# lmb-freiburg/flownet2

Hardware: AMD Instinct MI355X
Metric: image-pairs/sec FlowNetC forward at 448x320 (higher is better)
Workload: dtype f32

## Files before the change

flownet2_amd/csrc/conv_mfma.hip:

```cpp
#include "mfma_tile.hpp"

namespace fn2 {
namespace cv {

using namespace mfma;

struct Args {
  const float* in; const float* wp; const float* bias; float* out;
  int N, Cin, Hin, Win, in_ctot, in_c0;
  int Cout, Hout, Wout, out_ctot, out_c0;
  int pad;
  int nchunks;
  int ksteps;
  int tx, ty;
  int ng;
  unsigned total;
  unsigned nbig;
  float slope; int relu;
};

template <int KS_, int S_, int MW_, int NP_, int WM_, int WNX_, int WNY_, int CQ_, int P16_ = 0, int PIN_ = 0>
struct Cfg : Window<((P16_ ? 1 : 4) * WNY_ - 1) * S_ + KS_,
                    ((P16_ ? 16 : 4) * NP_ * WNX_ - 1) * S_ + KS_ + 4,
                    CQ_, WM_ * WNX_ * WNY_> {
  static constexpr int KS = KS_, S = S_, MW = MW_, NP = NP_, WM = WM_, WNX = WNX_, WNY = WNY_, CQ = CQ_, P16 = P16_;
  static constexpr int PIN = PIN_;
  static constexpr int NW = WM * WNX * WNY, THREADS = 64 * NW;
  static constexpr int PADL = 4;
  static constexpr int TW = (P16 ? 16 : 4) * NP * WNX, TH = (P16 ? 1 : 4) * WNY;
  static_assert(!P16 || (KS == 1 && S == 1), "row tiles are for 1x1 kernels");
  static_assert(Cfg::WR == (TH - 1) * S + KS && Cfg::WC == (TW - 1) * S + KS + PADL, "window of the tile");
  static constexpr int KSC = CQ * KS * KS;
  static constexpr int NBUFA = ring_depth(KSC);
  static_assert(KSC % NBUFA == 0, "ring phase must repeat per chunk");
  static_assert(2 * Cfg::BUF * 4 <= 160 * 1024, "LDS");
};

template <class K>
__device__ __forceinline__ void conv_body(const Args& a, int g, int bx, int by, int n) {
  static_assert(K::THREADS == 256, "launch bounds");
  extern __shared__ __attribute__((aligned(16))) float smem[];
  constexpr int KS = K::KS, S = K::S, MW = K::MW, NP = K::NP;
  const int tid = threadIdx.x, lane = tid & 63;
  const int wave = __builtin_amdgcn_readfirstlane(tid >> 6);
  const int wm = wave % K::WM, wnx = (wave / K::WM) % K::WNX, wny = wave / (K::WM * K::WNX);
  const int x0 = bx * K::TW, y0 = by * K::TH;

  const size_t plane = (size_t)a.Hin * a.Win;
  const __amdgpu_buffer_rsrc_t rs = nchw_rsrc(a.in, n, a.in_ctot, a.in_c0, a.Cin, plane);
  unsigned voff[K::RPW];
  window_plan<K>(voff, wave, lane, S * y0 - a.pad, S * x0 - K::PADL, a.Hin, a.Win, plane);
  const unsigned lds_base = (unsigned)(uintptr_t)(lds_ptr_t)smem;
  const unsigned chunk_bytes = 4u * 4u * K::CQ * (unsigned)plane;
  auto stage = [&](int chunk, int buf) { stage_chunk<K>(rs, voff, lds_base + 4u * (unsigned)(buf * K::BUF), wave, (unsigned)chunk * chunk_bytes); };

  const int kq = lane >> 4, p16 = lane & 15, py = K::P16 ? 0 : p16 >> 2, px = K::P16 ? p16 : p16 & 3;
  constexpr int PW = K::P16 ? 16 : 4, PH = K::P16 ? 1 : 4;
  const int bbase = kq * K::CS + (S * (PH * wny + py)) * K::RS + S * (PW * NP * wnx + px) + K::PADL - a.pad;
  using WV = typename WVec<MW>::T;
  const int cg0 = (g * K::WM + wm) * MW;
  const float* wb = a.wp + (size_t)(cg0 / 4) * a.ksteps * 256 + (cg0 % 4);
  const unsigned wlane = 16u * (unsigned)lane;

  f32x4 acc[MW][NP];
#pragma unroll
  for (int j = 0; j < MW; ++j)
#pragma unroll
    for (int p = 0; p < NP; ++p) acc[j][p] = f32x4{0.f, 0.f, 0.f, 0.f};

  constexpr int R = K::NBUFA - 1, DMA = K::NRUN / K::NW;
  static_assert(R + DMA <= 63, "vmcnt has 6 bits");
  WV wreg[K::NBUFA];
  stage(0, 0);
  if (a.nchunks > 0) {
#pragma unroll
    for (int i = 0; i < R; ++i) wreg[i] = weight_fetch<MW>(wb + (size_t)i * 256, wlane);
  }
  auto weight_step = [&](int ks0, int ks, int rest) -> WV {
    const float* wks = wb + (size_t)(ks0 + ks + R) * 256;
    if (ks + R < K::KSC) wreg[(ks + R) % K::NBUFA] = weight_fetch<MW>(wks, wlane);
    else wreg[(ks + R) % K::NBUFA] = weight_fetch_unless_last<MW>(rest, wks, wlane);
    const int left = K::KSC - 1 - ks < R ? K::KSC - 1 - ks : R;
    if (ks < R) ring_wait_either(rest, left, R + DMA);
    else if (left < R) ring_wait_either(rest, left, R);
    else ring_wait(R);
    weight_landed(wreg[ks % K::NBUFA]);
    return wreg[ks % K::NBUFA];
  };

  for (int c = 0; c < a.nchunks; ++c) {
    const int buf = c & 1;
    const int rest = a.nchunks - 1 - c;
    wait_vmcnt<R>();
    __builtin_amdgcn_s_barrier();
    if (rest) stage(c + 1, buf ^ 1);
    const float* win = smem + buf * K::BUF + bbase;
    const int ks0 = c * K::KSC;
    if constexpr (K::PIN) {
      float b[2][NP];
      auto tap_off = [](int ks) { const int cq = ks / (KS * KS), ky = (ks / KS) % KS, kx = ks % KS; return cq * 4 * K::CS + ky * K::RS + kx; };
#pragma unroll
      for (int p = 0; p < NP; ++p) b[0][p] = win[tap_off(0) + PW * S * p];
      __builtin_amdgcn_sched_barrier(0);
#pragma unroll
      for (int ks = 0; ks < K::KSC; ++ks) {
        const WV w = weight_step(ks0, ks, rest);
#pragma unroll
        for (int p = 0; p < NP; ++p) {
#pragma unroll
          for (int j = 0; j < MW; ++j) acc[j][p] = __builtin_amdgcn_mfma_f32_16x16x4f32(b[ks & 1][p], wget<MW>(w, j), acc[j][p], 0, 0, 0);
          if (ks + 1 < K::KSC) b[(ks + 1) & 1][p] = win[tap_off(ks + 1 < K::KSC ? ks + 1 : ks) + PW * S * p];
          __builtin_amdgcn_sched_barrier(0);
        }
      }
    } else {
#pragma unroll
    for (int ks = 0; ks < K::KSC; ++ks) {
      const WV w = weight_step(ks0, ks, rest);
      const int cq = ks / (KS * KS), ky = (ks / KS) % KS, kx = ks % KS;
      float b[NP];
#pragma unroll
      for (int p = 0; p < NP; ++p) b[p] = win[cq * 4 * K::CS + ky * K::RS + kx + PW * S * p];
#pragma unroll
      for (int j = 0; j < MW; ++j)
#pragma unroll
        for (int p = 0; p < NP; ++p) acc[j][p] = __builtin_amdgcn_mfma_f32_16x16x4f32(b[p], wget<MW>(w, j), acc[j][p], 0, 0, 0);
    }
    }
  }

  wait_vmcnt<0>();
  const int y = K::P16 ? y0 + wny : y0 + 4 * wny + (lane >> 4);
  if (y < a.Hout) {
#pragma unroll
    for (int j = 0; j < MW; ++j) {
      const int co = 16 * (cg0 + j) + (lane & 15);
      const float bv = a.bias ? a.bias[co] : 0.f;
      float* orow = a.out + (((size_t)n * a.out_ctot + a.out_c0 + co) * a.Hout + y) * a.Wout;
#pragma unroll
      for (int p = 0; p < NP; ++p) {
        const int x = K::P16 ? x0 + 16 * (NP * wnx + p) + 4 * (lane >> 4) : x0 + 4 * (NP * wnx + p);
        store_row4(orow, x, a.Wout, acc[j][p], bv, a.relu, a.slope);
      }
    }
  }
}

__device__ __forceinline__ void decode_tile(const Args& a, unsigned t, int& g, int& bx, int& by, int& n) {
  g = t % a.ng; t /= a.ng;
  bx = t % a.tx; t /= a.tx;
  by = t % a.ty;
  n = t / a.ty;
}

template <class K>
__global__ void __launch_bounds__(256, 2)
conv_mfma(Args a) {
  unsigned t;
  if (!xcd_task(blockIdx.x, a.total, t)) return;
  int g, bx, by, n;
  decode_tile(a, t, g, bx, by, n);
  conv_body<K>(a, g, bx, by, n);
}

template <class K>
__global__ void __launch_bounds__(256, 2)
conv_mfma_tail(Args a) {
  using KH = Cfg<K::KS, K::S, K::MW / 2, K::NP, K::WM, K::WNX, K::WNY, K::CQ, K::P16>;
  int g, bx, by, n;
  if (blockIdx.x < a.nbig) {
    const unsigned t = (blockIdx.x % 8) * (a.nbig / 8) + blockIdx.x / 8;
    decode_tile(a, t, g, bx, by, n);
    conv_body<K>(a, g, bx, by, n);
  } else {
    unsigned u;
    if (!xcd_task(blockIdx.x - a.nbig, 2 * (a.total - a.nbig), u)) return;
    decode_tile(a, a.nbig + u / 2, g, bx, by, n);
    conv_body<KH>(a, 2 * g + (int)(u & 1), bx, by, n);
  }
}

__global__ void pack_weights(const float* __restrict__ w, float* __restrict__ wp, int Cout, int Cin, int KS, int ksteps, int kalloc) {
  const long long total = (long long)((Cout + 63) / 64) * kalloc * 256;
  for (long long i = blockIdx.x * (long long)blockDim.x + threadIdx.x; i < total; i += (long long)gridDim.x * blockDim.x) {
    const int j = (int)(i & 3), lane = (int)((i >> 2) & 63);
    long long r = i >> 8;
    const int ks = (int)(r % kalloc), grp = (int)(r / kalloc);
    const int co = 64 * grp + 16 * j + (lane & 15), kq = lane >> 4;
    const int cq = ks / (KS * KS), tap = ks % (KS * KS);
    const int ci = 4 * cq + kq;
    float v = 0.f;
    if (ks < ksteps && ci < Cin && co < Cout) v = w[((size_t)co * Cin + ci) * KS * KS + tap];
    wp[i] = v;
  }
}

template <int KS> struct PackTile {
  static constexpr int T = KS * KS;
  static constexpr int QT = KS == 1 ? 8 : KS == 3 ? 3 : KS == 4 ? 2 : 1;
  static constexpr int CIL = 4 * QT, ROW = CIL * T + 1;
  static constexpr int LDS_FLOATS = 64 * ROW;
};

template <int KS, int ORDER>
__global__ void __launch_bounds__(256) pack_weights_view(const float* __restrict__ w, float* __restrict__ wp, int ksteps, int kalloc,
                                                         int src_co, int src_ci, long long s_co, long long s_ci, int flip) {
  using P = PackTile<KS>;
  constexpr int T = P::T, QT = P::QT, CIL = P::CIL, ROW = P::ROW;
  __shared__ float tile[P::LDS_FLOATS];
  const int grp = blockIdx.x, cq0 = blockIdx.y * QT;
  const int co0 = 64 * grp, ci0 = 4 * cq0;
  const int nquads = ksteps / T;
  constexpr int TOTAL = 64 * CIL * T;
  if constexpr (ORDER == 0) {
    const float* src = w + (size_t)co0 * s_co + (size_t)ci0 * T;
#pragma unroll
    for (int i = threadIdx.x; i < TOTAL; i += 256) {
      const int col = i / (CIL * T), e = i - col * (CIL * T), c = e / T;
      tile[col * ROW + e] = (co0 + col < src_co && ci0 + c < src_ci) ? src[(size_t)col * s_co + e] : 0.f;
    }
  } else if constexpr (ORDER == 1) {
    const float* src = w + (size_t)ci0 * s_ci + (size_t)co0 * T;
#pragma unroll
    for (int i = threadIdx.x; i < TOTAL; i += 256) {
      const int c = i / (64 * T), e = i - c * (64 * T), col = e / T, t = e - col * T;
      tile[col * ROW + c * T + t] = (co0 + col < src_co && ci0 + c < src_ci) ? src[(size_t)c * s_ci + e] : 0.f;
    }
  } else {
#pragma unroll
    for (int i = threadIdx.x; i < TOTAL; i += 256) {
      const int col = i / (CIL * T), e = i - col * (CIL * T), c = e / T, t = e - c * T;
      tile[col * ROW + e] = (co0 + col < src_co && ci0 + c < src_ci) ? w[(size_t)(co0 + col) * s_co + (size_t)(ci0 + c) * s_ci + t] : 0.f;
    }
  }
  __syncthreads();
  const int nq = min(QT, nquads - cq0);
  float* dst = wp + ((size_t)grp * kalloc + (size_t)cq0 * T) * 256;
  const int j = threadIdx.x & 3, lane = threadIdx.x >> 2;
  const float* trow = tile + (16 * j + (lane & 15)) * ROW + (lane >> 4) * T;
#pragma unroll
  for (int ks = 0; ks < QT * T; ++ks) {
    const int cq = ks / T, tap = ks - cq * T;
    if (cq < nq) dst[ks * 256 + threadIdx.x] = trow[4 * cq * T + (flip ? T - 1 - tap : tap)];
  }
  if (cq0 + QT >= nquads)
    for (int i = threadIdx.x; i < (kalloc - ksteps) * 256; i += 256) wp[((size_t)grp * kalloc + ksteps) * 256 + i] = 0.f;
}

template <int KS>
static void launch_pack_view(const float* w, float* wp, int Cout, int ksteps, int kalloc, int src_co, int src_ci, long long s_co, long long s_ci, int flip,
                             hipStream_t st) {
  using P = PackTile<KS>;
  const dim3 grid((unsigned)((Cout + 63) / 64), (unsigned)cdiv(ksteps / P::T, P::QT));
  if (s_ci == (long long)P::T) hipLaunchKernelGGL((pack_weights_view<KS, 0>), grid, dim3(256), 0, st, w, wp, ksteps, kalloc, src_co, src_ci, s_co, s_ci, flip);
  else if (s_co == (long long)P::T) hipLaunchKernelGGL((pack_weights_view<KS, 1>), grid, dim3(256), 0, st, w, wp, ksteps, kalloc, src_co, src_ci, s_co, s_ci, flip);
  else hipLaunchKernelGGL((pack_weights_view<KS, 2>), grid, dim3(256), 0, st, w, wp, ksteps, kalloc, src_co, src_ci, s_co, s_ci, flip);
}

constexpr int kSpare = 8;
constexpr int kChunkQuads = 2;

inline int chunk_quads(int KS) { return KS == 1 ? 8 : kChunkQuads; }
inline int ksteps_for(int Cin, int KS) { return cdiv(cdiv(Cin, 4), chunk_quads(KS)) * chunk_quads(KS) * KS * KS; }

template <class K>
static void set_geometry(Args& a) {
  if constexpr (K::P16) {
    a.Win *= a.Hin; a.Hin = 1; a.Wout *= a.Hout; a.Hout = 1;
  }
  a.tx = cdiv(a.Wout, K::TW); a.ty = cdiv(a.Hout, K::TH);
  a.ng = a.Cout / (16 * K::MW * K::WM);
  a.nchunks = cdiv(cdiv(a.Cin, 4), K::CQ);
}

inline long long tiles_of(const Args& a) { return (long long)a.N * a.tx * a.ty * a.ng; }

template <class K>
static int launch(const Args& base, hipStream_t st) {
  Args a = base;
  set_geometry<K>(a);
  a.nbig = (unsigned)tiles_of(a);
  return launch_tiles<&conv_mfma<K>>(a, tiles_of(a), K::THREADS, (int)(sizeof(float) * 2 * K::BUF), "conv_mfma", "conv_mfma_forward", st);
}

inline unsigned whole_rounds(long long tiles) { return (unsigned)(tiles / 256 * 256); }

template <class K>
static int launch_tail(const Args& base, hipStream_t st) {
  if constexpr (K::MW < 2) {
    return fail(FN2_ERR_UNSUPPORTED, "conv_mfma: variant has no split tail");
  } else {
    Args a = base;
    set_geometry<K>(a);
    if (tiles_of(a) > 0x1fffff00ll) return fail(FN2_ERR_UNSUPPORTED, "conv_mfma: grid too large");
    a.total = (unsigned)tiles_of(a); a.nbig = whole_rounds(a.total);
    const unsigned nsm = 2 * (a.total - a.nbig);
    const unsigned grid = a.nbig + 8 * ((nsm + 7) / 8);
    constexpr size_t lds = sizeof(float) * 2 * K::BUF;
    set_dynamic_lds_once<&conv_mfma_tail<K>>((int)lds);
    hipLaunchKernelGGL((conv_mfma_tail<K>), dim3(grid), dim3(K::THREADS), lds, st, a);
    return check_launch("conv_mfma_forward");
  }
}

struct Variant {
  int ks, s, mw, np, wm, wnx, wny, p16;
  int (*fn)(const Args&, hipStream_t);
  int (*fn_tail)(const Args&, hipStream_t);
};

#define FN2_CV_LIST(X) \
   \
  X(1, 1, 2, 7, 2, 2, 1, 8, 1) X(1, 1, 2, 7, 2, 1, 2, 8, 1) X(1, 1, 4, 7, 1, 2, 2, 8, 0) X(1, 1, 4, 7, 1, 1, 4, 8, 0) X(1, 1, 2, 6, 2, 2, 1, 8, 1) \
  X(1, 1, 2, 4, 2, 2, 1, 8, 1) X(1, 1, 2, 7, 1, 2, 2, 8, 0) X(1, 1, 2, 7, 1, 4, 1, 8, 0) X(1, 1, 2, 4, 1, 2, 2, 8, 0) X(1, 1, 4, 4, 1, 2, 2, 8, 0) \
   \
  X(3, 1, 2, 7, 2, 2, 1, 2, 1) X(3, 1, 2, 7, 2, 1, 2, 2, 1) X(3, 1, 4, 7, 1, 2, 2, 2, 0) X(3, 1, 4, 7, 1, 1, 4, 2, 0) \
  X(3, 1, 2, 6, 2, 2, 1, 2, 1) X(3, 1, 4, 6, 1, 2, 2, 2, 0) X(3, 1, 4, 4, 1, 2, 2, 2, 0) X(3, 1, 2, 4, 2, 2, 1, 2, 1) \
   \
  X(3, 2, 2, 7, 2, 1, 2, 2, 1) X(3, 2, 4, 7, 1, 1, 4, 2, 0) X(3, 2, 2, 6, 2, 2, 1, 2, 1) X(3, 2, 4, 6, 1, 2, 2, 2, 0) X(3, 2, 2, 4, 2, 2, 1, 2, 1) \
   \
  X(4, 2, 2, 7, 2, 2, 1, 2, 1) X(4, 2, 2, 7, 2, 1, 2, 2, 1) X(4, 2, 4, 7, 1, 2, 2, 2, 0) X(4, 2, 2, 6, 2, 2, 1, 2, 1) X(4, 2, 4, 4, 1, 2, 2, 2, 0) X(4, 2, 2, 4, 2, 2, 1, 2, 1) \
   \
  X(5, 2, 2, 7, 2, 2, 1, 1, 1) X(5, 2, 2, 7, 2, 1, 2, 1, 1) X(5, 2, 4, 7, 1, 2, 2, 1, 0) X(5, 2, 4, 7, 1, 1, 4, 1, 0) \
  X(5, 2, 2, 6, 2, 2, 1, 1, 1) X(5, 2, 4, 6, 1, 2, 2, 1, 0) X(5, 2, 4, 4, 1, 2, 2, 1, 0) \
   \
  X(7, 2, 2, 6, 2, 2, 1, 1, 1) X(7, 2, 2, 7, 2, 2, 1, 1, 1) X(7, 2, 4, 4, 1, 2, 2, 1, 0) X(7, 2, 4, 6, 1, 2, 2, 1, 0) X(7, 2, 2, 4, 2, 2, 1, 1, 1)

template <class K, int TAIL> struct TailFn { static constexpr int (*fn)(const Args&, hipStream_t) = nullptr; };
template <class K> struct TailFn<K, 1> { static constexpr int (*fn)(const Args&, hipStream_t) = &launch_tail<K>; };

#define FN2_CV_ROW(KS, S, MW, NP, WM, WNX, WNY, CQ, TAIL) \
  {KS, S, MW, NP, WM, WNX, WNY, 0, &launch<Cfg<KS, S, MW, NP, WM, WNX, WNY, CQ>>, TailFn<Cfg<KS, S, MW, NP, WM, WNX, WNY, CQ>, TAIL>::fn},
#define FN2_CV_ROW16(MW, NP, WM, WNX, WNY, TAIL) \
  {1, 1, MW, NP, WM, WNX, WNY, 1, &launch<Cfg<1, 1, MW, NP, WM, WNX, WNY, 8, 1>>, TailFn<Cfg<1, 1, MW, NP, WM, WNX, WNY, 8, 1>, TAIL>::fn},
#define FN2_CV_PIN(KS, S, MW, NP, WM, WNX, WNY, CQ, P16, TAIL) \
  {KS, S, MW, NP, WM, WNX, WNY, P16, &launch<Cfg<KS, S, MW, NP, WM, WNX, WNY, CQ, P16, 1>>, TailFn<Cfg<KS, S, MW, NP, WM, WNX, WNY, CQ, P16, 1>, TAIL>::fn},
static const Variant kVariants[] = {FN2_CV_LIST(FN2_CV_ROW)
  FN2_CV_ROW16(2, 7, 2, 2, 1, 1) FN2_CV_ROW16(2, 7, 4, 1, 1, 1) FN2_CV_ROW16(4, 7, 1, 4, 1, 0) FN2_CV_ROW16(4, 7, 2, 2, 1, 0) FN2_CV_ROW16(2, 5, 2, 2, 1, 1)
  FN2_CV_ROW16(2, 4, 2, 2, 1, 1) FN2_CV_ROW16(2, 7, 1, 4, 1, 0) FN2_CV_ROW16(2, 5, 1, 4, 1, 0) FN2_CV_ROW16(4, 5, 1, 4, 1, 0) FN2_CV_ROW16(2, 4, 1, 4, 1, 0)
  FN2_CV_ROW16(4, 5, 2, 2, 1, 0) FN2_CV_ROW16(4, 4, 2, 2, 1, 0)
  FN2_CV_ROW16(2, 9, 4, 1, 1, 1) FN2_CV_ROW16(2, 9, 2, 2, 1, 1) FN2_CV_ROW16(2, 3, 2, 2, 1, 1) FN2_CV_ROW16(4, 3, 1, 4, 1, 0)
  FN2_CV_ROW16(4, 9, 4, 1, 1, 0) FN2_CV_ROW16(4, 9, 2, 2, 1, 0) FN2_CV_ROW16(4, 7, 4, 1, 1, 0)
  FN2_CV_PIN(5, 2, 2, 7, 2, 2, 1, 1, 0, 1) FN2_CV_PIN(5, 2, 2, 7, 2, 1, 2, 1, 0, 1)
  FN2_CV_PIN(1, 1, 4, 9, 4, 1, 1, 8, 1, 0) FN2_CV_PIN(1, 1, 2, 9, 4, 1, 1, 8, 1, 1) FN2_CV_PIN(1, 1, 2, 5, 2, 2, 1, 8, 1, 1) FN2_CV_PIN(1, 1, 4, 7, 4, 1, 1, 8, 1, 0)
  FN2_CV_PIN(1, 1, 2, 7, 2, 2, 1, 8, 1, 1) FN2_CV_PIN(1, 1, 2, 3, 2, 2, 1, 8, 1, 1)
  FN2_CV_PIN(3, 1, 2, 7, 2, 2, 1, 2, 0, 1) FN2_CV_PIN(3, 1, 2, 6, 2, 2, 1, 2, 0, 1) FN2_CV_PIN(3, 2, 2, 7, 2, 1, 2, 2, 0, 1) FN2_CV_PIN(3, 2, 2, 6, 2, 2, 1, 2, 0, 1)
  FN2_CV_PIN(4, 2, 2, 7, 2, 2, 1, 2, 0, 1) FN2_CV_PIN(4, 2, 2, 6, 2, 2, 1, 2, 0, 1) FN2_CV_PIN(5, 2, 2, 6, 2, 2, 1, 1, 0, 1)
  FN2_CV_PIN(7, 2, 2, 6, 2, 2, 1, 1, 0, 1) FN2_CV_PIN(7, 2, 4, 6, 1, 2, 2, 1, 0, 0)};
constexpr int kNumVariants = sizeof(kVariants) / sizeof(kVariants[0]);

int g_forced_variant = -1;

static double variant_cost(const Variant& v, const Args& a, bool tail) {
  const int tw = (v.p16 ? 16 : 4) * v.np * v.wnx, th = (v.p16 ? 1 : 4) * v.wny;
  const long long wgs = v.p16 ? (long long)a.N * cdiv(a.Wout * a.Hout, tw) * (a.Cout / (16 * v.mw * v.wm))
                              : (long long)a.N * cdiv(a.Wout, tw) * cdiv(a.Hout, th) * (a.Cout / (16 * v.mw * v.wm));
  double rounds = (double)((wgs + 255) / 256);
  if (tail) {
    const long long r = wgs % 256;
    if (wgs < 256 || r == 0 || r > 128) return 1e30;
    rounds = (double)(wgs / 256) + 0.5 * 1.12;
  }
  const double eff = 1.0 / (1.0 + 0.08 * (4.0 / v.mw - 1.0) + 0.02 * (7.0 / v.np - 1.0));
  return rounds * v.mw * v.np / eff;
}

static bool variant_applies(const Variant& v, const Args& a, int KS, int S) {
  if (!v.p16 && a.Win % 4 != 0) return false;
  return v.ks == KS && v.s == S && a.Cout % (16 * v.mw * v.wm) == 0;
}

}
}

using namespace fn2;

FN2_API size_t fn2_conv_mfma_packed_floats(int Cout, int Cin, int kernel) {
  if (Cout <= 0 || Cout % 32 != 0 || Cin <= 0 || kernel <= 0) return 0;
  return (size_t)((Cout + 63) / 64) * (cv::ksteps_for(Cin, kernel) + cv::kSpare) * 256;
}

FN2_API int fn2_conv_mfma_pack_weights_view(const float* weight, float* packed, int Cout, int Cin, int kernel, int src_cout, int src_cin,
                                            long long stride_cout, long long stride_cin, int flip, void* stream);

FN2_API int fn2_conv_mfma_pack_weights(const float* weight, float* packed, int Cout, int Cin, int kernel, void* stream) {
  if (!weight || !packed) return fail(FN2_ERR_INVALID_ARG, "conv_mfma_pack_weights: null blob");
  if (Cout <= 0 || Cout % 32 != 0 || Cin <= 0 || (kernel != 1 && kernel != 3 && kernel != 4 && kernel != 5 && kernel != 7))
    return fail(FN2_ERR_UNSUPPORTED, "conv_mfma_pack_weights: needs Cout %% 32 == 0 and kernel_size 1, 3, 4, 5 or 7 (got Cout %d, kernel %d)", Cout, kernel);
  return fn2_conv_mfma_pack_weights_view(weight, packed, Cout, Cin, kernel, Cout, Cin, (long long)Cin * kernel * kernel, (long long)kernel * kernel, 0, stream);
}

FN2_API int fn2_conv_mfma_pack_weights_view(const float* weight, float* packed, int Cout, int Cin, int kernel, int src_cout, int src_cin,
                                            long long stride_cout, long long stride_cin, int flip, void* stream) {
  if (!weight || !packed) return fail(FN2_ERR_INVALID_ARG, "conv_mfma_pack_weights_view: null blob");
  if (Cout <= 0 || Cout % 32 != 0 || Cin <= 0 || (kernel != 1 && kernel != 3 && kernel != 4 && kernel != 5 && kernel != 7))
    return fail(FN2_ERR_UNSUPPORTED, "conv_mfma_pack_weights_view: needs Cout %% 32 == 0 and kernel_size 1, 3, 4, 5 or 7 (got Cout %d, kernel %d)", Cout, kernel);
  if (src_cout < 1 || src_cout > Cout || src_cin < 1 || src_cin > Cin || stride_cout < 1 || stride_cin < 1)
    return fail(FN2_ERR_INVALID_ARG, "conv_mfma_pack_weights_view: bad source view (%d of %d, %d of %d channels, strides %lld / %lld)", src_cout, Cout,
                src_cin, Cin, stride_cout, stride_cin);
  const int ksteps = cv::ksteps_for(Cin, kernel), kalloc = ksteps + cv::kSpare;
  hipStream_t st = as_stream(stream);
  switch (kernel) {
    case 1: cv::launch_pack_view<1>(weight, packed, Cout, ksteps, kalloc, src_cout, src_cin, stride_cout, stride_cin, flip ? 1 : 0, st); break;
    case 3: cv::launch_pack_view<3>(weight, packed, Cout, ksteps, kalloc, src_cout, src_cin, stride_cout, stride_cin, flip ? 1 : 0, st); break;
    case 4: cv::launch_pack_view<4>(weight, packed, Cout, ksteps, kalloc, src_cout, src_cin, stride_cout, stride_cin, flip ? 1 : 0, st); break;
    case 5: cv::launch_pack_view<5>(weight, packed, Cout, ksteps, kalloc, src_cout, src_cin, stride_cout, stride_cin, flip ? 1 : 0, st); break;
    default: cv::launch_pack_view<7>(weight, packed, Cout, ksteps, kalloc, src_cout, src_cin, stride_cout, stride_cin, flip ? 1 : 0, st); break;
  }
  return check_launch("conv_mfma_pack_weights_view");
}

FN2_API int fn2_conv_mfma_supported(int Cin, int Hin, int Win, int Cout, int kernel, int stride, int pad) {
  if (Cin <= 0 || Hin <= 0 || Win <= 0 || Cout <= 0 || Cout % 32 != 0) return 0;
  if (kernel == 1 ? ((long long)Hin * Win) % 4 != 0 : Win % 4 != 0) return 0;
  if (!((kernel == 1 && stride == 1) || (kernel == 3 && (stride == 1 || stride == 2)) || (kernel == 4 && stride == 2) || (kernel == 5 && stride == 2) || (kernel == 7 && stride == 2))) return 0;
  if (pad < 0 || pad > 4 || pad > kernel - 1) return 0;
  if ((long long)Cin * Hin * Win >= (1ll << 28)) return 0;
  const int Hout = (Hin + 2 * pad - kernel) / stride + 1, Wout = (Win + 2 * pad - kernel) / stride + 1;
  if (Hout < 1 || Wout < 1) return 0;
  cv::Args a{};
  a.Win = Win; a.Cout = Cout;
  for (int i = 0; i < cv::kNumVariants; ++i)
    if (cv::variant_applies(cv::kVariants[i], a, kernel, stride)) return 1;
  return 0;
}

FN2_API int fn2_debug_set_conv_variant(int v) { cv::g_forced_variant = v; return FN2_OK; }
FN2_API int fn2_conv_mfma_num_variants(void) { return cv::kNumVariants; }

FN2_API int fn2_conv_mfma_forward(const float* bottom, const float* packed_weight, const float* bias, float* top,
                                  int N, int Cin, int Hin, int Win, int bottom_channels, int bottom_c0,
                                  int Cout, int top_channels, int top_c0, int kernel, int stride, int pad,
                                  int relu, float negative_slope, void* stream) {
  if (N < 0) return fail(FN2_ERR_INVALID_ARG, "conv_mfma: bad batch");
  if (N == 0) return FN2_OK;
  if (const int rc = mfma::check_conv_args("conv_mfma", bottom, packed_weight, top, Cin, bottom_channels, bottom_c0, Cout, top_channels, top_c0, [&] {
        return fn2_conv_mfma_supported(Cin, Hin, Win, Cout, kernel, stride, pad) ? FN2_OK
            : fail(FN2_ERR_UNSUPPORTED, "conv_mfma: unsupported geometry (Cin %d, %dx%d, Cout %d, k %d s %d p %d)", Cin, Hin, Win, Cout, kernel, stride, pad);
      }))
    return rc;
  cv::Args a{};
  a.in = bottom; a.wp = packed_weight; a.bias = bias; a.out = top;
  a.N = N; a.Cin = Cin; a.Hin = Hin; a.Win = Win; a.in_ctot = bottom_channels; a.in_c0 = bottom_c0;
  a.Cout = Cout; a.Hout = (Hin + 2 * pad - kernel) / stride + 1; a.Wout = (Win + 2 * pad - kernel) / stride + 1;
  a.out_ctot = top_channels; a.out_c0 = top_c0; a.pad = pad;
  a.ksteps = cv::ksteps_for(Cin, kernel) + cv::kSpare;
  a.slope = negative_slope; a.relu = relu;
  hipStream_t st = as_stream(stream);
  static TuneCache cache("conv_mfma", cv::kNumVariants);
  const TuneKey key{N, Cin, Hin, Win, Cout, kernel, stride, pad, bottom_channels == Cin, top_channels == Cout};
  mfma::Pick p;
  if (const int rc = mfma::pick_variant(p, "conv_mfma", cv::g_forced_variant, cv::kNumVariants, true, cache, key, st,
                                        [&](int i) { return cv::variant_applies(cv::kVariants[i], a, kernel, stride); },
                                        [&](int i, bool tail) { return cv::variant_cost(cv::kVariants[i], a, tail); },
                                        [&](int i, bool tail) { return tail ? cv::kVariants[i].fn_tail(a, st) : cv::kVariants[i].fn(a, st); },
                                        [&](int i) { return cv::kVariants[i].fn_tail != nullptr; }))
    return rc;
  return p.tail ? cv::kVariants[p.variant].fn_tail(a, st) : cv::kVariants[p.variant].fn(a, st);
}
```

flownet2_amd/csrc/mfma_tile.hpp:

```cpp
#pragma once

#include "autotune.hpp"
#include "fn2_common.hpp"

namespace fn2 {
namespace mfma {

using f32x4 = __attribute__((ext_vector_type(4))) float;
using f32x2 = __attribute__((ext_vector_type(2))) float;
using lds_ptr_t = __attribute__((address_space(3))) void*;

constexpr int cdiv(int a, int b) { return (a + b - 1) / b; }
constexpr int up_mod(int v, int r, int m) { return v + ((r - v % m) + m) % m; }

constexpr unsigned kOOB = 0x7ffffff0u;
constexpr int kRsrcWord3 = 0x00020000;

template <int N>
__device__ __forceinline__ void wait_vmcnt() {
  asm volatile("s_waitcnt vmcnt(%0)" ::"n"(N) : "memory");
}

__device__ __forceinline__ __amdgpu_buffer_rsrc_t nchw_rsrc(const float* blob, int n, int ctot, int c0, int C, size_t plane) {
  return __builtin_amdgcn_make_buffer_rsrc(const_cast<float*>(blob + ((size_t)n * ctot + c0) * plane), 0, (unsigned)(4u * C * plane), kRsrcWord3);
}

template <int MW> struct WVec;
template <> struct WVec<1> { using T = float; };
template <> struct WVec<2> { using T = f32x2; };
template <> struct WVec<4> { using T = f32x4; };

template <int MW>
__device__ __forceinline__ float wget(const typename WVec<MW>::T& v, int j) {
  if constexpr (MW == 1) return v; else return v[j];
}

template <int WR_, int WC_, int CQ_, int NW_>
struct Window {
  static constexpr int WR = WR_, WC = WC_;
  static constexpr int RS = up_mod(cdiv(WC, 4) * 4, 4, 16);
  static constexpr int CS = up_mod(WR * RS, 16, 32);
  static constexpr int SLOTS_C = CS / 4;
  static constexpr int SLOTS = 4 * CQ_ * SLOTS_C;
  static constexpr int NRUN = cdiv(SLOTS, 64);
  static constexpr int RPW = cdiv(NRUN, NW_);
  static constexpr int BUF = NRUN * 256;
};

constexpr int ring_depth(int KSC) { return (KSC % 6 == 0) ? 6 : (KSC % 5 == 0) ? 5 : (KSC % 7 == 0) ? 7 : (KSC % 4 == 0) ? 4 : 3; }

template <class K>
__device__ __forceinline__ void window_plan(unsigned (&voff)[K::RPW], int wave, int lane, int y_first, int x_first, int Hin, int Win, size_t plane) {
#pragma unroll
  for (int i = 0; i < K::RPW; ++i) {
    const int s = (i * K::NW + wave) * 64 + lane;
    voff[i] = kOOB;
    if (s < K::SLOTS) {
      const int c = s / K::SLOTS_C, rem = s % K::SLOTS_C;
      const int row = rem / (K::RS / 4), gq = rem % (K::RS / 4);
      const int yi = y_first + row, xi = x_first + 4 * gq;
      if (row < K::WR && 4 * gq < K::WC && yi >= 0 && yi < Hin && xi >= 0 && xi < Win)
        voff[i] = 4u * (unsigned)(c * plane + (size_t)yi * Win + xi);
    }
  }
}

template <class K>
__device__ __forceinline__ void stage_chunk(__amdgpu_buffer_rsrc_t rs, const unsigned (&voff)[K::RPW], unsigned dst, int wave, unsigned soff) {
#pragma unroll
  for (int i = 0; i < K::RPW; ++i) {
    const int r = i * K::NW + wave;
    if (r < K::NRUN)
      __builtin_amdgcn_raw_ptr_buffer_load_lds(rs, (lds_ptr_t)(uintptr_t)(dst + 1024u * (unsigned)r), 16, voff[i], soff, 0, 0);
  }
}

template <class K>
struct ChunkStage {
  const __amdgpu_buffer_rsrc_t& rs; const unsigned (&voff)[K::RPW]; const unsigned& chunk_bytes; const unsigned& dst; const int& wave;
  __device__ void operator()(int chunk) const {
    unsigned vc[K::RPW];
#pragma unroll
    for (int i = 0; i < K::RPW; ++i) vc[i] = voff[i] == kOOB ? kOOB : voff[i] + (unsigned)chunk * chunk_bytes;
    stage_chunk<K>(rs, vc, dst, wave, 0u);
  }
};

__device__ __forceinline__ const float* weight_lane(const float* wp, int cg0, int ksteps, int lane) {
  return wp + ((size_t)(cg0 / 4) * ksteps * 64 + lane) * 4 + (cg0 % 4);
}

template <int MW>
__device__ __forceinline__ typename WVec<MW>::T weight_load(const float* wl, int ks) {
  return *reinterpret_cast<const typename WVec<MW>::T*>(wl + (size_t)ks * 256);
}

template <int MW>
__device__ __forceinline__ typename WVec<MW>::T weight_fetch(const float* base, unsigned lane_bytes) {
  typename WVec<MW>::T w;
  if constexpr (MW == 1) asm volatile("global_load_dword %0, %1, %2" : "=v"(w) : "v"(lane_bytes), "s"(base));
  else if constexpr (MW == 2) asm volatile("global_load_dwordx2 %0, %1, %2" : "=v"(w) : "v"(lane_bytes), "s"(base));
  else asm volatile("global_load_dwordx4 %0, %1, %2" : "=v"(w) : "v"(lane_bytes), "s"(base));
  return w;
}

template <class T>
__device__ __forceinline__ void weight_landed(T& w) { asm volatile("" : "+v"(w)); }

constexpr int vmcnt_clamp(int n) { return n < 63 ? n : 63; }

__device__ __forceinline__ void ring_wait(int n) { asm volatile("s_waitcnt vmcnt(%0)" ::"i"(vmcnt_clamp(n))); }

__device__ __forceinline__ void ring_wait_either(int rest, int n_last, int n_else) {
  asm volatile(
      "s_cmp_eq_u32 %0, 0\n\t"
      "s_cbranch_scc1 .Lrwt_%=\n\t"
      "s_waitcnt vmcnt(%2)\n\t"
      "s_branch .Lrwe_%=\n"
      ".Lrwt_%=:\n\t"
      "s_waitcnt vmcnt(%1)\n"
      ".Lrwe_%=:"
      :
      : "s"(rest), "i"(vmcnt_clamp(n_last)), "i"(vmcnt_clamp(n_else))
      : "scc");
}

template <int MW>
__device__ __forceinline__ typename WVec<MW>::T weight_fetch_unless_last(int rest, const float* base, unsigned lane_bytes) {
  typename WVec<MW>::T w;
#define FN2_FETCH_UNLESS(INSN) \
  asm volatile("s_cmp_eq_u32 %3, 0\n\ts_cbranch_scc1 .Lwfs_%=\n\t" INSN " %0, %1, %2\n.Lwfs_%=:" : "=v"(w) : "v"(lane_bytes), "s"(base), "s"(rest) : "scc")
  if constexpr (MW == 1) FN2_FETCH_UNLESS("global_load_dword");
  else if constexpr (MW == 2) FN2_FETCH_UNLESS("global_load_dwordx2");
  else FN2_FETCH_UNLESS("global_load_dwordx4");
#undef FN2_FETCH_UNLESS
  return w;
}

__device__ __forceinline__ bool xcd_task(unsigned block, unsigned total, unsigned& task) {
  const unsigned per_xcd = (total + 7) / 8;
  task = (block % 8) * per_xcd + block / 8;
  return !(block / 8 >= per_xcd || task >= total);
}

__device__ __forceinline__ f32x4 bias_relu4(f32x4 v, float bias, int relu, float slope) {
#pragma unroll
  for (int r = 0; r < 4; ++r) {
    float s = v[r] + bias;
    if (relu) s = s > 0.f ? s : s * slope;
    v[r] = s;
  }
  return v;
}

__device__ __forceinline__ void store4(float* orow, int x, int Wout, f32x4 v) {
  if (x + 3 < Wout) *reinterpret_cast<f32x4*>(orow + x) = v;
  else {
#pragma unroll
    for (int r = 0; r < 4; ++r) if (x + r < Wout) orow[x + r] = v[r];
  }
}

__device__ __forceinline__ void store_row4(float* orow, int x, int Wout, f32x4 v, float bias, int relu, float slope) {
  store4(orow, x, Wout, bias_relu4(v, bias, relu, slope));
}

template <auto Kernel>
inline void set_dynamic_lds_once(int bytes) {
  static bool attr_set = false;
  if (!attr_set) {
    (void)hipFuncSetAttribute(reinterpret_cast<const void*>(Kernel), hipFuncAttributeMaxDynamicSharedMemorySize, bytes);
    attr_set = true;
  }
}

template <auto Kernel, class Args>
int launch_tiles(Args& a, long long tiles, int threads, int lds_bytes, const char* what, const char* checked, hipStream_t st) {
  if (tiles > 0x3fffff00ll) return fail(FN2_ERR_UNSUPPORTED, "%s: grid too large", what);
  a.total = (unsigned)tiles;
  set_dynamic_lds_once<Kernel>(lds_bytes);
  hipLaunchKernelGGL(Kernel, dim3(8 * ((a.total + 7) / 8)), dim3(threads), lds_bytes, st, a);
  return check_launch(checked);
}

template <class Geometry>
int check_conv_args(const char* what, const float* bottom, const float* packed, const float* top, int Cin, int bottom_channels, int bottom_c0,
                    int Cout, int top_channels, int top_c0, Geometry geometry) {
  if (!bottom || !packed || !top) return fail(FN2_ERR_INVALID_ARG, "%s: null blob", what);
  if (const int rc = geometry()) return rc;
  if (bottom_c0 < 0 || bottom_c0 + Cin > bottom_channels || top_c0 < 0 || top_c0 + Cout > top_channels)
    return fail(FN2_ERR_INVALID_ARG, "%s: channel slice outside the blob", what);
  if (((reinterpret_cast<uintptr_t>(bottom) | reinterpret_cast<uintptr_t>(top) | reinterpret_cast<uintptr_t>(packed)) & 15) != 0)
    return fail(FN2_ERR_UNSUPPORTED, "%s: blobs must be 16-byte aligned", what);
  return FN2_OK;
}

struct Pick { int variant = -1; bool tail = false; };

template <class Applies, class Cost, class Run, class HasTail>
int pick_variant(Pick& p, const char* what, int forced, int nvariants, bool split_tail, TuneCache& cache, const TuneKey& key, hipStream_t st,
                 Applies applies, Cost cost, Run run, HasTail has_tail) {
  p = Pick{};
  if (forced >= 0) {
    p.tail = split_tail && forced >= 1000;
    p.variant = split_tail ? forced % 1000 : forced;
    if (p.variant >= nvariants || !applies(p.variant) || (p.tail && !has_tail(p.variant)))
      return fail(FN2_ERR_UNSUPPORTED, "%s: forced variant %d does not apply", what, forced);
    return FN2_OK;
  }
  int picked = -1;
  if (autotune_enabled(st)) {
    auto usable = [&](int c) -> bool {
      const int i = split_tail ? c / 2 : c;
      return applies(i) && (!(split_tail && (c & 1)) || (has_tail(i) && cost(i, true) < 1e29));
    };
    picked = autotune_pick(cache, key, split_tail ? 2 * nvariants : nvariants, st, [&](int c) -> int {
      return usable(c) ? run(split_tail ? c / 2 : c, split_tail && (c & 1)) : FN2_ERR_UNSUPPORTED;
    }, usable);
  }
  if (picked >= 0) {
    p.variant = split_tail ? picked / 2 : picked;
    p.tail = split_tail && (picked & 1);
  } else {
    double bc = 0;
    for (int i = 0; i < nvariants; ++i) {
      if (!applies(i)) continue;
      for (int t = 0; t < (split_tail && has_tail(i) ? 2 : 1); ++t) {
        const double c = cost(i, t == 1);
        if (p.variant < 0 || c < bc) { p.variant = i; bc = c; p.tail = t == 1; }
      }
    }
  }
  if (p.variant < 0) return fail(FN2_ERR_UNSUPPORTED, "%s: no kernel variant for this geometry", what);
  return FN2_OK;
}

}
}
```

Baseline: 3595.

## Skip padded k-steps in last chunk, add small 1x1 variant and cost floor

The conv MFMA kernel now computes how many k-steps are real in the final channel chunk (klast) and skips the MFMA and LDS reads for padded quads beyond it, cutting wasted work when Cin/4 is not a multiple of the chunk size. A new narrow 1x1 row variant (NP=1) is added, and the heuristic cost model gains a per-round floor so tiny variants are not over-favoured on small layers. The model selection is factored out and exposed through a debug entry point. The runtime branch on klast may add some control overhead or disturb the instruction scheduling inside the unrolled loop.

```diff
diff --git a/flownet2_amd/csrc/conv_mfma.hip b/flownet2_amd/csrc/conv_mfma.hip
--- a/flownet2_amd/csrc/conv_mfma.hip
+++ b/flownet2_amd/csrc/conv_mfma.hip
@@ -11,6 +11,7 @@
   int Cout, Hout, Wout, out_ctot, out_c0;
   int pad;
   int nchunks;
+  int klast;
   int ksteps;
   int tx, ty;
   int ng;
@@ -96,6 +97,9 @@
     if (rest) stage(c + 1, buf ^ 1);
     const float* win = smem + buf * K::BUF + bbase;
     const int ks0 = c * K::KSC;
+    constexpr int T = KS * KS;
+    const int kend = rest ? K::KSC : a.klast;
+    auto live = [&](int ks) { return ks < T || ks < kend; };
     if constexpr (K::PIN) {
       float b[2][NP];
       auto tap_off = [](int ks) { const int cq = ks / (KS * KS), ky = (ks / KS) % KS, kx = ks % KS; return cq * 4 * K::CS + ky * K::RS + kx; };
@@ -105,26 +109,30 @@
 #pragma unroll
       for (int ks = 0; ks < K::KSC; ++ks) {
         const WV w = weight_step(ks0, ks, rest);
-#pragma unroll
-        for (int p = 0; p < NP; ++p) {
-#pragma unroll
-          for (int j = 0; j < MW; ++j) acc[j][p] = __builtin_amdgcn_mfma_f32_16x16x4f32(b[ks & 1][p], wget<MW>(w, j), acc[j][p], 0, 0, 0);
-          if (ks + 1 < K::KSC) b[(ks + 1) & 1][p] = win[tap_off(ks + 1 < K::KSC ? ks + 1 : ks) + PW * S * p];
-          __builtin_amdgcn_sched_barrier(0);
+        if (live(ks)) {
+#pragma unroll
+          for (int p = 0; p < NP; ++p) {
+#pragma unroll
+            for (int j = 0; j < MW; ++j) acc[j][p] = __builtin_amdgcn_mfma_f32_16x16x4f32(b[ks & 1][p], wget<MW>(w, j), acc[j][p], 0, 0, 0);
+            if (ks + 1 < K::KSC) b[(ks + 1) & 1][p] = win[tap_off(ks + 1 < K::KSC ? ks + 1 : ks) + PW * S * p];
+            __builtin_amdgcn_sched_barrier(0);
+          }
         }
       }
     } else {
 #pragma unroll
     for (int ks = 0; ks < K::KSC; ++ks) {
       const WV w = weight_step(ks0, ks, rest);
-      const int cq = ks / (KS * KS), ky = (ks / KS) % KS, kx = ks % KS;
-      float b[NP];
-#pragma unroll
-      for (int p = 0; p < NP; ++p) b[p] = win[cq * 4 * K::CS + ky * K::RS + kx + PW * S * p];
-#pragma unroll
-      for (int j = 0; j < MW; ++j)
-#pragma unroll
-        for (int p = 0; p < NP; ++p) acc[j][p] = __builtin_amdgcn_mfma_f32_16x16x4f32(b[p], wget<MW>(w, j), acc[j][p], 0, 0, 0);
+      if (live(ks)) {
+        const int cq = ks / (KS * KS), ky = (ks / KS) % KS, kx = ks % KS;
+        float b[NP];
+#pragma unroll
+        for (int p = 0; p < NP; ++p) b[p] = win[cq * 4 * K::CS + ky * K::RS + kx + PW * S * p];
+#pragma unroll
+        for (int j = 0; j < MW; ++j)
+#pragma unroll
+          for (int p = 0; p < NP; ++p) acc[j][p] = __builtin_amdgcn_mfma_f32_16x16x4f32(b[p], wget<MW>(w, j), acc[j][p], 0, 0, 0);
+      }
     }
     }
   }
@@ -271,6 +279,7 @@
   a.tx = cdiv(a.Wout, K::TW); a.ty = cdiv(a.Hout, K::TH);
   a.ng = a.Cout / (16 * K::MW * K::WM);
   a.nchunks = cdiv(cdiv(a.Cin, 4), K::CQ);
+  a.klast = (cdiv(a.Cin, 4) - (a.nchunks - 1) * K::CQ) * K::KS * K::KS;
 }
 
 inline long long tiles_of(const Args& a) { return (long long)a.N * a.tx * a.ty * a.ng; }
@@ -346,11 +355,13 @@
   FN2_CV_PIN(1, 1, 2, 7, 2, 2, 1, 8, 1, 1) FN2_CV_PIN(1, 1, 2, 3, 2, 2, 1, 8, 1, 1)
   FN2_CV_PIN(3, 1, 2, 7, 2, 2, 1, 2, 0, 1) FN2_CV_PIN(3, 1, 2, 6, 2, 2, 1, 2, 0, 1) FN2_CV_PIN(3, 2, 2, 7, 2, 1, 2, 2, 0, 1) FN2_CV_PIN(3, 2, 2, 6, 2, 2, 1, 2, 0, 1)
   FN2_CV_PIN(4, 2, 2, 7, 2, 2, 1, 2, 0, 1) FN2_CV_PIN(4, 2, 2, 6, 2, 2, 1, 2, 0, 1) FN2_CV_PIN(5, 2, 2, 6, 2, 2, 1, 1, 0, 1)
-  FN2_CV_PIN(7, 2, 2, 6, 2, 2, 1, 1, 0, 1) FN2_CV_PIN(7, 2, 4, 6, 1, 2, 2, 1, 0, 0)};
+  FN2_CV_PIN(7, 2, 2, 6, 2, 2, 1, 1, 0, 1) FN2_CV_PIN(7, 2, 4, 6, 1, 2, 2, 1, 0, 0)
+  FN2_CV_ROW16(2, 1, 1, 4, 1, 1)};
 constexpr int kNumVariants = sizeof(kVariants) / sizeof(kVariants[0]);
 
 int g_forced_variant = -1;
 
+constexpr double kStepFloor = 6.0;
 static double variant_cost(const Variant& v, const Args& a, bool tail) {
   const int tw = (v.p16 ? 16 : 4) * v.np * v.wnx, th = (v.p16 ? 1 : 4) * v.wny;
   const long long wgs = v.p16 ? (long long)a.N * cdiv(a.Wout * a.Hout, tw) * (a.Cout / (16 * v.mw * v.wm))
@@ -362,12 +373,23 @@
     rounds = (double)(wgs / 256) + 0.5 * 1.12;
   }
   const double eff = 1.0 / (1.0 + 0.08 * (4.0 / v.mw - 1.0) + 0.02 * (7.0 / v.np - 1.0));
-  return rounds * v.mw * v.np / eff;
+  const double work = rounds * v.mw * v.np / eff;
+  const double floor = kStepFloor * (double)(((wgs + 255) / 256 + 1) / 2);
+  return work > floor ? work : floor;
 }
 
 static bool variant_applies(const Variant& v, const Args& a, int KS, int S) {
   if (!v.p16 && a.Win % 4 != 0) return false;
   return v.ks == KS && v.s == S && a.Cout % (16 * v.mw * v.wm) == 0;
+}
+
+static Args layer_args(int N, int Cin, int Hin, int Win, int Cout, int kernel, int stride, int pad) {
+  Args a{};
+  a.N = N; a.Cin = Cin; a.Hin = Hin; a.Win = Win;
+  a.Cout = Cout; a.Hout = (Hin + 2 * pad - kernel) / stride + 1; a.Wout = (Win + 2 * pad - kernel) / stride + 1;
+  a.pad = pad;
+  a.ksteps = ksteps_for(Cin, kernel) + kSpare;
+  return a;
 }
 
 }
@@ -428,6 +450,16 @@
 FN2_API int fn2_debug_set_conv_variant(int v) { cv::g_forced_variant = v; return FN2_OK; }
 FN2_API int fn2_conv_mfma_num_variants(void) { return cv::kNumVariants; }
 
+FN2_API int fn2_debug_conv_mfma_model_pick(int N, int Cin, int Hin, int Win, int Cout, int kernel, int stride, int pad) {
+  if (N <= 0 || !fn2_conv_mfma_supported(Cin, Hin, Win, Cout, kernel, stride, pad)) return -1;
+  const cv::Args a = cv::layer_args(N, Cin, Hin, Win, Cout, kernel, stride, pad);
+  mfma::Pick p;
+  mfma::model_pick(p, cv::kNumVariants, true, [&](int i) { return cv::variant_applies(cv::kVariants[i], a, kernel, stride); },
+                   [&](int i, bool tail) { return cv::variant_cost(cv::kVariants[i], a, tail); },
+                   [&](int i) { return cv::kVariants[i].fn_tail != nullptr; });
+  return p.variant < 0 ? -1 : p.variant + (p.tail ? 1000 : 0);
+}
+
 FN2_API int fn2_conv_mfma_forward(const float* bottom, const float* packed_weight, const float* bias, float* top,
                                   int N, int Cin, int Hin, int Win, int bottom_channels, int bottom_c0,
                                   int Cout, int top_channels, int top_c0, int kernel, int stride, int pad,
@@ -439,12 +471,9 @@
             : fail(FN2_ERR_UNSUPPORTED, "conv_mfma: unsupported geometry (Cin %d, %dx%d, Cout %d, k %d s %d p %d)", Cin, Hin, Win, Cout, kernel, stride, pad);
       }))
     return rc;
-  cv::Args a{};
+  cv::Args a = cv::layer_args(N, Cin, Hin, Win, Cout, kernel, stride, pad);
   a.in = bottom; a.wp = packed_weight; a.bias = bias; a.out = top;
-  a.N = N; a.Cin = Cin; a.Hin = Hin; a.Win = Win; a.in_ctot = bottom_channels; a.in_c0 = bottom_c0;
-  a.Cout = Cout; a.Hout = (Hin + 2 * pad - kernel) / stride + 1; a.Wout = (Win + 2 * pad - kernel) / stride + 1;
-  a.out_ctot = top_channels; a.out_c0 = top_c0; a.pad = pad;
-  a.ksteps = cv::ksteps_for(Cin, kernel) + cv::kSpare;
+  a.in_ctot = bottom_channels; a.in_c0 = bottom_c0; a.out_ctot = top_channels; a.out_c0 = top_c0;
   a.slope = negative_slope; a.relu = relu;
   hipStream_t st = as_stream(stream);
   static TuneCache cache("conv_mfma", cv::kNumVariants);
diff --git a/flownet2_amd/csrc/mfma_tile.hpp b/flownet2_amd/csrc/mfma_tile.hpp
--- a/flownet2_amd/csrc/mfma_tile.hpp
+++ b/flownet2_amd/csrc/mfma_tile.hpp
@@ -197,6 +197,19 @@
 
 struct Pick { int variant = -1; bool tail = false; };
 
+template <class Applies, class Cost, class HasTail>
+void model_pick(Pick& p, int nvariants, bool split_tail, Applies applies, Cost cost, HasTail has_tail) {
+  p = Pick{};
+  double bc = 0;
+  for (int i = 0; i < nvariants; ++i) {
+    if (!applies(i)) continue;
+    for (int t = 0; t < (split_tail && has_tail(i) ? 2 : 1); ++t) {
+      const double c = cost(i, t == 1);
+      if (p.variant < 0 || c < bc) { p.variant = i; bc = c; p.tail = t == 1; }
+    }
+  }
+}
+
 template <class Applies, class Cost, class Run, class HasTail>
 int pick_variant(Pick& p, const char* what, int forced, int nvariants, bool split_tail, TuneCache& cache, const TuneKey& key, hipStream_t st,
                  Applies applies, Cost cost, Run run, HasTail has_tail) {
@@ -222,14 +235,7 @@
     p.variant = split_tail ? picked / 2 : picked;
     p.tail = split_tail && (picked & 1);
   } else {
-    double bc = 0;
-    for (int i = 0; i < nvariants; ++i) {
-      if (!applies(i)) continue;
-      for (int t = 0; t < (split_tail && has_tail(i) ? 2 : 1); ++t) {
-        const double c = cost(i, t == 1);
-        if (p.variant < 0 || c < bc) { p.variant = i; bc = c; p.tail = t == 1; }
-      }
-    }
+    model_pick(p, nvariants, split_tail, applies, cost, has_tail);
   }
   if (p.variant < 0) return fail(FN2_ERR_UNSUPPORTED, "%s: no kernel variant for this geometry", what);
   return FN2_OK;
```

Result: no change. 3616, median of 6 (+0.6%).
